# seorim0/DNN-based-Speech-Enhancement-in-the-frequency-domain

Hardware: AMD Instinct MI355X
Metric: train utts/sec (3s@16kHz) DCCRN (higher is better)
Workload: dtype bf16; 1 GPU; DCCRN mask C, SI-SNR, fwd+bwd+Adam, B=32/GPU x 3s@16kHz clips (BASELINE configs[1]); global_batch=32, parallelism=dp1, bn=per-rank statistics, collective=none

## Files before the change

dnn-based-speech-enhancement-in-the-frequency-domain_amd/csrc/bn.hip:

```cpp
#include <hip/hip_runtime.h>
#include <cstdlib>
#include "sefd_desc.h"
#include "tuning.h"
#include "dev_common.h"

namespace sefd {

template <typename T> struct VecIO;
template <> struct VecIO<float> {
  static constexpr int V = 4;
  static __device__ __forceinline__ void load(const char* base, int64_t i, float* o) {
    const float4 v = *reinterpret_cast<const float4*>(base + i * 4);
    o[0] = v.x; o[1] = v.y; o[2] = v.z; o[3] = v.w;
  }
  static __device__ __forceinline__ void store(char* base, int64_t i, const float* o) {
    *reinterpret_cast<float4*>(base + i * 4) = make_float4(o[0], o[1], o[2], o[3]);
  }
};
template <> struct VecIO<bf16_t> {
  static constexpr int V = 8;
  static __device__ __forceinline__ void load(const char* base, int64_t i, float* o) {
    const uint4 v = *reinterpret_cast<const uint4*>(base + i * 2);
    const uint32_t w[4] = {v.x, v.y, v.z, v.w};
#pragma unroll
    for (int k = 0; k < 4; ++k) { o[2 * k] = bf2f(w[k] & 0xffff); o[2 * k + 1] = bf2f(w[k] >> 16); }
  }
  static __device__ __forceinline__ void store(char* base, int64_t i, const float* o) {
    uint4 v;
    v.x = pack_bf16x2(o[0], o[1]); v.y = pack_bf16x2(o[2], o[3]);
    v.z = pack_bf16x2(o[4], o[5]); v.w = pack_bf16x2(o[6], o[7]);
    *reinterpret_cast<uint4*>(base + i * 2) = v;
  }
};

constexpr int kMaxC = kBnMaxC;
static_assert(kMaxC <= 1024, "bn_bwd_reduce_kernel_v: red[512 * V + 8] holds 256 V channels x 2 sums, and C / V chunk columns must fit 256 threads in fp32");

__device__ __forceinline__ void stage_params(float* sp, int C, const float* mi, const float* gamma, const float* beta) {
  for (int c = threadIdx.x; c < C; c += blockDim.x) { sp[c] = mi[c]; sp[C + c] = mi[C + c]; sp[2 * C + c] = gamma[c]; sp[3 * C + c] = beta[c]; }
  __syncthreads();
}

template <typename T>
__global__ __launch_bounds__(256) void bn_apply_kernel_v(const BnApply d, const ArenaBases ab, const int rev) {
  constexpr int V = VecIO<T>::V;
  __shared__ float sp[4 * kMaxC];
  const int C = d.C;
  stage_params(sp, C, reinterpret_cast<const float*>(rp(ab, d.mean_invstd)), reinterpret_cast<const float*>(rp(ab, d.gamma)),
               reinterpret_cast<const float*>(rp(ab, d.beta)));
  const char* y = rp(ab, d.y);
  char* z = rp(ab, d.z);
  const float a = *reinterpret_cast<const float*>(rp(ab, d.slope));
  const int cmask = (C & (C - 1)) == 0 ? C - 1 : -1;
  const int64_t nq = d.R * C / V;
  const int64_t stride = (int64_t)gridDim.x * blockDim.x;
  if (cmask >= 0 && ((stride * V) & cmask) == 0) {
    const int64_t idx0 = blockIdx.x * (int64_t)blockDim.x + threadIdx.x;
    const int c = (int)(((rev ? nq - 1 - idx0 : idx0) * V) & cmask);
    float pm[V], pis[V], pg[V], pb[V];
#pragma unroll
    for (int e = 0; e < V; ++e) { pm[e] = sp[c + e]; pis[e] = sp[C + c + e]; pg[e] = sp[2 * C + c + e]; pb[e] = sp[3 * C + c + e]; }
    for (int64_t qq = idx0; qq < nq; qq += stride) {
      const int64_t q = rev ? nq - 1 - qq : qq;
      float v[V];
      VecIO<T>::load(y, q * V, v);
#pragma unroll
      for (int e = 0; e < V; ++e) {
        const float bn = pg[e] * ((v[e] - pm[e]) * pis[e]) + pb[e];
        v[e] = bn > 0.f ? bn : a * bn;
      }
      VecIO<T>::store(z, q * V, v);
    }
    return;
  }
  for (int64_t q = blockIdx.x * (int64_t)blockDim.x + threadIdx.x; q < nq; q += stride) {
    const int64_t i = q * V;
    const int c = cmask >= 0 ? (int)(i & cmask) : (int)(i % C);
    float v[V];
    VecIO<T>::load(y, i, v);
#pragma unroll
    for (int e = 0; e < V; ++e) {
      const float bn = sp[2 * C + c + e] * ((v[e] - sp[c + e]) * sp[C + c + e]) + sp[3 * C + c + e];
      v[e] = bn > 0.f ? bn : a * bn;
    }
    VecIO<T>::store(z, i, v);
  }
}

template <typename T>
__device__ __forceinline__ void load_dz_v(const BnBwdReduce& d, const char* dz0, const char* dz1, int64_t b, int ql, int c, float* g) {
  constexpr int V = VecIO<T>::V;
#pragma unroll
  for (int e = 0; e < V; ++e) g[e] = 0.f;
  if (ql >= d.skip) VecIO<T>::load(dz0, (b * (d.rpb - d.skip) + ql - d.skip) * d.C + c, g);
  if (dz1) {
    float h[V];
    VecIO<T>::load(dz1, (b * d.rpb + ql) * d.C + c, h);
#pragma unroll
    for (int e = 0; e < V; ++e) g[e] += h[e];
  }
}

template <typename T>
__global__ __launch_bounds__(256) void bn_bwd_reduce_kernel_v(const BnBwdReduce d, const ArenaBases ab, const int rev) {
  constexpr int V = VecIO<T>::V;
  __shared__ float sp[4 * kMaxC];
  __shared__ float red[512 * V + 8];
  const int C = d.C;
  stage_params(sp, C, reinterpret_cast<const float*>(rp(ab, d.mean_invstd)), reinterpret_cast<const float*>(rp(ab, d.gamma)),
               reinterpret_cast<const float*>(rp(ab, d.beta)));
  const char* y = rp(ab, d.y);
  const char* dz0 = rp(ab, d.dz0);
  const char* dz1 = d.dz1.arena >= 0 ? rp(ab, d.dz1) : nullptr;
  const float a = *reinterpret_cast<const float*>(rp(ab, d.slope));
  const int CV = C / V;
  const int nrl = 256 / CV > 0 ? 256 / CV : 1;
  const int rl = threadIdx.x / CV, cc = threadIdx.x - rl * CV;
  float s0[V], s1[V], sa = 0.f;
#pragma unroll
  for (int e = 0; e < V; ++e) { s0[e] = 0.f; s1[e] = 0.f; }
  const int blk = rev ? (int)gridDim.x - 1 - (int)blockIdx.x : (int)blockIdx.x;
  const int64_t row0 = (int64_t)blk * d.rows_per_blk;
  const int64_t row1 = min(d.R, row0 + d.rows_per_blk);
  if (rl < nrl && cc < CV) {
    const int c = cc * V;
    float pm[V], pis[V], pg[V], pb[V];
#pragma unroll
    for (int e = 0; e < V; ++e) { pm[e] = sp[c + e]; pis[e] = sp[C + c + e]; pg[e] = sp[2 * C + c + e]; pb[e] = sp[3 * C + c + e]; }
    int64_t r = row0 + rl;
    int64_t b = r / d.rpb;
    int ql = (int)(r - b * d.rpb);
    auto accumulate = [&](const float* yv, const float* gz) {
#pragma unroll
      for (int e = 0; e < V; ++e) {
        const float xh = (yv[e] - pm[e]) * pis[e];
        const float bn = pg[e] * xh + pb[e];
        const float dbn = bn > 0.f ? gz[e] : a * gz[e];
        sa += bn > 0.f ? 0.f : bn * gz[e];
        s0[e] += dbn;
        s1[e] += dbn * xh;
      }
    };
    auto next_row = [&]() { r += nrl; ql += nrl; while (ql >= d.rpb) { ql -= (int)d.rpb; ++b; } };
    while (r + nrl < row1) {
      float yv0[V], gz0[V], yv1[V], gz1[V];
      VecIO<T>::load(y, r * C + c, yv0);
      load_dz_v<T>(d, dz0, dz1, b, ql, c, gz0);
      next_row();
      VecIO<T>::load(y, r * C + c, yv1);
      load_dz_v<T>(d, dz0, dz1, b, ql, c, gz1);
      next_row();
      accumulate(yv0, gz0);
      accumulate(yv1, gz1);
    }
    if (r < row1) {
      float yv[V], gz[V];
      VecIO<T>::load(y, r * C + c, yv);
      load_dz_v<T>(d, dz0, dz1, b, ql, c, gz);
      accumulate(yv, gz);
    }
#pragma unroll
    for (int e = 0; e < V; ++e) {
      red[(rl * C + c + e) * 2 + 0] = s0[e];
      red[(rl * C + c + e) * 2 + 1] = s1[e];
    }
  }
  __syncthreads();
  float* part = reinterpret_cast<float*>(rp(ab, d.part)) + (int64_t)blk * 3 * C;
  for (int c = threadIdx.x; c < C; c += 256) {
    float t0 = 0.f, t1 = 0.f;
    for (int k = 0; k < nrl; ++k) { t0 += red[(k * C + c) * 2 + 0]; t1 += red[(k * C + c) * 2 + 1]; }
    part[c] = t0;
    part[C + c] = t1;
  }
  __syncthreads();
  sa = wave_sum(sa);
  if ((threadIdx.x & 63) == 0) red[512 * V + (threadIdx.x >> 6)] = sa;
  __syncthreads();
  if (threadIdx.x == 0) part[2 * C] = red[512 * V] + red[512 * V + 1] + red[512 * V + 2] + red[512 * V + 3];
  for (int c = 1 + threadIdx.x; c < C; c += 256) part[2 * C + c] = 0.f;
}

template <typename T>
__global__ __launch_bounds__(256) void bn_bwd_apply_kernel_v(const BnBwdApply d, const ArenaBases ab) {
  constexpr int V = VecIO<T>::V;
  __shared__ float sp[4 * kMaxC];
  __shared__ float st[2 * kMaxC];
  const BnBwdReduce& r = d.r;
  const int C = r.C;
  stage_params(sp, C, reinterpret_cast<const float*>(rp(ab, r.mean_invstd)), reinterpret_cast<const float*>(rp(ab, r.gamma)),
               reinterpret_cast<const float*>(rp(ab, r.beta)));
  const float* tot = reinterpret_cast<const float*>(rp(ab, d.totals));
  const float inv_n = (float)(1.0 / d.count);
  for (int c = threadIdx.x; c < C; c += blockDim.x) { st[c] = tot[c] * inv_n; st[C + c] = tot[C + c] * inv_n; }
  __syncthreads();
  const char* y = rp(ab, r.y);
  const char* dz0 = rp(ab, r.dz0);
  const char* dz1 = r.dz1.arena >= 0 ? rp(ab, r.dz1) : nullptr;
  char* dy = rp(ab, d.dy);
  const float a = *reinterpret_cast<const float*>(rp(ab, r.slope));
  const int64_t b = blockIdx.y;
  const int nq = (int)(r.rpb * C / V);
  const int cmask = (C & (C - 1)) == 0 ? C - 1 : -1;
  const int csh = cmask >= 0 ? __ffs(C) - 1 : 0;
  const int qstride = gridDim.x * blockDim.x;
  if (cmask >= 0 && ((qstride * V) & cmask) == 0) {
    const int c = ((blockIdx.x * blockDim.x + threadIdx.x) * V) & cmask;
    float pm[V], pis[V], pg[V], pb[V], t0[V], t1[V];
#pragma unroll
    for (int e = 0; e < V; ++e) {
      pm[e] = sp[c + e]; pis[e] = sp[C + c + e]; pg[e] = sp[2 * C + c + e]; pb[e] = sp[3 * C + c + e];
      t0[e] = st[c + e]; t1[e] = st[C + c + e];
    }
    for (int q = blockIdx.x * blockDim.x + threadIdx.x; q < nq; q += qstride) {
      const int il = q * V;
      const int ql = il >> csh;
      float yv[V], gz[V], o[V];
      const int64_t gi = b * r.rpb * C + il;
      VecIO<T>::load(y, gi, yv);
      load_dz_v<T>(r, dz0, dz1, b, ql, c, gz);
#pragma unroll
      for (int e = 0; e < V; ++e) {
        const float xh = (yv[e] - pm[e]) * pis[e];
        const float bn = pg[e] * xh + pb[e];
        const float dbn = bn > 0.f ? gz[e] : a * gz[e];
        o[e] = pg[e] * pis[e] * (dbn - t0[e] - xh * t1[e]);
      }
      VecIO<T>::store(dy, gi, o);
    }
    return;
  }
  for (int q = blockIdx.x * blockDim.x + threadIdx.x; q < nq; q += qstride) {
    const int il = q * V;
    const int ql = cmask >= 0 ? (il >> csh) : il / C;
    const int c = il - ql * C;
    float yv[V], gz[V], o[V];
    const int64_t gi = b * r.rpb * C + il;
    VecIO<T>::load(y, gi, yv);
    load_dz_v<T>(r, dz0, dz1, b, ql, c, gz);
#pragma unroll
    for (int e = 0; e < V; ++e) {
      const float xh = (yv[e] - sp[c + e]) * sp[C + c + e];
      const float bn = sp[2 * C + c + e] * xh + sp[3 * C + c + e];
      const float dbn = bn > 0.f ? gz[e] : a * gz[e];
      o[e] = sp[2 * C + c + e] * sp[C + c + e] * (dbn - st[c + e] - xh * st[C + c + e]);
    }
    VecIO<T>::store(dy, gi, o);
  }
}

static inline int gridcap(int64_t n, int cap = 16384) {
  int64_t g = (n + 255) / 256;
  return (int)(g < 1 ? 1 : (g > cap ? cap : g));
}

void launch_bn(const Op& op, const ArenaBases& ab, hipStream_t st) {
  constexpr int rev = 1;
  if (op.kind == OP_BN_APPLY) {
    const BnApply& d = op.bna;
    if (d.dt == DT_BF16) hipLaunchKernelGGL((bn_apply_kernel_v<bf16_t>), dim3(gridcap(d.R * d.C / 8)), dim3(256), 0, st, d, ab, rev);
    else hipLaunchKernelGGL((bn_apply_kernel_v<float>), dim3(gridcap(d.R * d.C / 4)), dim3(256), 0, st, d, ab, rev);
  } else if (op.kind == OP_BN_BWD_REDUCE) {
    const BnBwdReduce& d = op.bnr;
    if (d.dt == DT_BF16) hipLaunchKernelGGL((bn_bwd_reduce_kernel_v<bf16_t>), dim3(d.nblk), dim3(256), 0, st, d, ab, rev);
    else hipLaunchKernelGGL((bn_bwd_reduce_kernel_v<float>), dim3(d.nblk), dim3(256), 0, st, d, ab, rev);
  } else if (op.kind == OP_BN_BWD_APPLY) {
    const BnBwdApply& d = op.bnb;
    const int nb = (int)(d.r.R / d.r.rpb);
    const int v = d.r.dt == DT_BF16 ? 8 : 4;
    int gx = gridcap(d.r.rpb * d.r.C / v, 16384 / (nb > 0 ? nb : 1) + 1);
    if (d.r.dt == DT_BF16) hipLaunchKernelGGL((bn_bwd_apply_kernel_v<bf16_t>), dim3(gx, nb), dim3(256), 0, st, d, ab);
    else hipLaunchKernelGGL((bn_bwd_apply_kernel_v<float>), dim3(gx, nb), dim3(256), 0, st, d, ab);
  }
}

}
```

dnn-based-speech-enhancement-in-the-frequency-domain_amd/csrc/kernels.hip:

```cpp
#include <hip/hip_runtime.h>
#include <algorithm>
#include <mutex>
#include <unordered_map>
#include "sefd_desc.h"
#include "tuning.h"
#include "dev_common.h"

namespace sefd {

static inline int cdiv64(int64_t a, int64_t b) { return (int)((a + b - 1) / b); }
static inline int grid_for(int64_t n, int block = 256, int cap = 8192) {
  int64_t g = (n + block - 1) / block;
  return (int)(g < 1 ? 1 : (g > cap ? cap : g));
}

__global__ void pack_kernel(const Pack d, const ArenaBases ab) {
  const int32_t* tab = reinterpret_cast<const int32_t*>(rp(ab, d.tab));
  const float* src = reinterpret_cast<const float*>(rp(ab, d.src));
  char* dst = rp(ab, d.dst);
  for (int64_t i = blockIdx.x * (int64_t)blockDim.x + threadIdx.x; i < d.n; i += (int64_t)gridDim.x * blockDim.x) {
    float v = 0.f;
    for (int e = 0; e < d.width; ++e) {
      const int32_t t = tab[i * d.width + e];
      if (t > 0) v += src[t - 1];
      else if (t < 0) v -= src[-t - 1];
    }
    st_elem(dst, d.ddt, i, v);
  }
}

__global__ void packmulti_kernel(const PackMulti m, const ArenaBases ab) {
  const Pack d = reinterpret_cast<const Pack*>(rp(ab, m.entries))[blockIdx.y];
  const int32_t* tab = reinterpret_cast<const int32_t*>(rp(ab, d.tab));
  const float* src = reinterpret_cast<const float*>(rp(ab, d.src));
  char* dst = rp(ab, d.dst);
  for (int64_t i = blockIdx.x * (int64_t)blockDim.x + threadIdx.x; i < d.n; i += (int64_t)gridDim.x * blockDim.x) {
    float v = 0.f;
    for (int e = 0; e < d.width; ++e) {
      const int32_t t = tab[i * d.width + e];
      if (t > 0) v += src[t - 1];
      else if (t < 0) v -= src[-t - 1];
    }
    st_elem(dst, d.ddt, i, v);
  }
}

__global__ __launch_bounds__(256) void splitsum_kernel(Unpack d, const ArenaBases ab) {
  __shared__ float4 red[16][16];
  float* part = reinterpret_cast<float*>(rp(ab, d.part));
  if (d.nseg > 0) {
    const int64_t* seg = reinterpret_cast<const int64_t*>(rp(ab, d.start)) + 3 * (int64_t)blockIdx.y;
    part += seg[0];
    d.n = d.sstride = seg[1];
    d.nsplit = (int32_t)seg[2];
  }
  const int ex = threadIdx.x & 15, sy = threadIdx.x >> 4;
  const bool vec = (d.n & 3) == 0 && (d.sstride & 3) == 0 && (reinterpret_cast<uintptr_t>(part) & 15) == 0;
  for (int64_t base = (int64_t)blockIdx.x * 64; base < d.n; base += (int64_t)gridDim.x * 64) {
    const int64_t i = base + ex * 4;
    float4 s = make_float4(0.f, 0.f, 0.f, 0.f);
    if (vec) {
      if (i < d.n)
        for (int k = sy; k < d.nsplit; k += 16) {
          const float4 v = *reinterpret_cast<const float4*>(part + (int64_t)k * d.sstride + i);
          s.x += v.x; s.y += v.y; s.z += v.z; s.w += v.w;
        }
    } else {
      float* sp = &s.x;
      for (int e = 0; e < 4; ++e)
        if (i + e < d.n)
          for (int k = sy; k < d.nsplit; k += 16) sp[e] += part[(int64_t)k * d.sstride + i + e];
    }
    red[sy][ex] = s;
    __syncthreads();
    if (sy == 0) {
      float4 t = red[0][ex];
#pragma unroll
      for (int j = 1; j < 16; ++j) { const float4 v = red[j][ex]; t.x += v.x; t.y += v.y; t.z += v.z; t.w += v.w; }
      if (vec) { if (i < d.n) *reinterpret_cast<float4*>(part + i) = t; }
      else { const float* tp = &t.x; for (int e = 0; e < 4; ++e) if (i + e < d.n) part[i + e] = tp[e]; }
    }
    __syncthreads();
  }
}

__global__ void unpack_kernel(const Unpack d, const ArenaBases ab) {
  const int32_t* start = reinterpret_cast<const int32_t*>(rp(ab, d.start));
  const int32_t* ent = reinterpret_cast<const int32_t*>(rp(ab, d.ent));
  const float* part = reinterpret_cast<const float*>(rp(ab, d.part));
  float* dst = reinterpret_cast<float*>(rp(ab, d.dst));
  for (int64_t j = blockIdx.x * (int64_t)blockDim.x + threadIdx.x; j < d.n; j += (int64_t)gridDim.x * blockDim.x) {
    float v = 0.f;
    for (int e = start[j]; e < start[j + 1]; ++e) {
      const int32_t t = ent[e];
      if (t > 0) v += part[t - 1];
      else if (t < 0) v -= part[-t - 1];
    }
    if (start[j + 1] > start[j]) dst[j] = v;
  }
}

__global__ __launch_bounds__(256) void bn_finalize_kernel(const BnFinalize d, const ArenaBases ab) {
  const int c = blockIdx.x;
  if (d.nblk < 0) {
    if (threadIdx.x == 0) {
      float* mi = reinterpret_cast<float*>(rp(ab, d.mean_invstd));
      mi[c] = reinterpret_cast<const float*>(rp(ab, d.running_mean))[c];
      mi[d.C + c] = 1.f / sqrtf(reinterpret_cast<const float*>(rp(ab, d.running_var))[c] + d.eps);
    }
    return;
  }
  const float* part = reinterpret_cast<const float*>(rp(ab, d.part));
  __shared__ double r1[256], r2[256];
  if (d.mode == 2) {
    if (threadIdx.x == 0) {
      const double* tot = reinterpret_cast<const double*>(rp(ab, d.totals));
      r1[0] = tot[c];
      r2[0] = tot[d.C + c];
    }
  } else {
    double s1 = 0.0, s2 = 0.0;
    const int nsub = d.nsub > 1 ? d.nsub : 1;
    for (int b = threadIdx.x; b < d.nblk; b += 256)
      for (int u = 0; u < nsub; ++u) {
        s1 += part[((int64_t)b * 2 + 0) * d.Cpad + u * d.substride + c];
        s2 += part[((int64_t)b * 2 + 1) * d.Cpad + u * d.substride + c];
      }
    r1[threadIdx.x] = s1;
    r2[threadIdx.x] = s2;
    __syncthreads();
    for (int o = 128; o > 0; o >>= 1) {
      if (threadIdx.x < o) { r1[threadIdx.x] += r1[threadIdx.x + o]; r2[threadIdx.x] += r2[threadIdx.x + o]; }
      __syncthreads();
    }
    if (d.mode == 1) {
      if (threadIdx.x == 0) {
        double* tot = reinterpret_cast<double*>(rp(ab, d.totals));
        tot[c] = r1[0];
        tot[d.C + c] = r2[0];
      }
      return;
    }
  }
  if (threadIdx.x == 0) {
    const double mean = r1[0] / d.count;
    double var = r2[0] / d.count - mean * mean;
    if (var < 0) var = 0;
    float* mi = reinterpret_cast<float*>(rp(ab, d.mean_invstd));
    mi[c] = (float)mean;
    mi[d.C + c] = (float)(1.0 / sqrt(var + (double)d.eps));
    if (d.running_mean.arena >= 0) {
      float* rm = reinterpret_cast<float*>(rp(ab, d.running_mean));
      float* rv = reinterpret_cast<float*>(rp(ab, d.running_var));
      const double unb = var * (d.count / (d.count > 1 ? d.count - 1 : 1));
      rm[c] = (float)((1.0 - d.momentum) * rm[c] + d.momentum * mean);
// ... 389 lines not shown
    float v = 0.f;
    if (k >= 0 && k < d.NF) {
      const float sr = spec[(f * NS + k + 1) * 2], si = spec[(f * NS + k + 1) * 2 + 1];
      v = sqrtf(sr * sr + si * si);
    }
    st_elem(mags, d.dt, i, v);
  }
}

__global__ void specpad_kernel(const Mags d, const ArenaBases ab) {
  const float* spec = reinterpret_cast<const float*>(rp(ab, d.spec));
  char* out = rp(ab, d.mags);
  const int64_t n = d.frames * d.NF * d.MS;
  for (int64_t i = blockIdx.x * (int64_t)blockDim.x + threadIdx.x; i < n; i += (int64_t)gridDim.x * blockDim.x) {
    const int ch = (int)(i % d.MS);
    const int64_t slot = i / d.MS;
    st_elem(out, d.dt, i, ch < 2 ? spec[slot * 2 + ch] : 0.f);
  }
}

__global__ void ola_fwd_kernel(const Ola d, const ArenaBases ab) {
  const float* fr = reinterpret_cast<const float*>(rp(ab, d.frames));
  const float* coff = reinterpret_cast<const float*>(rp(ab, d.coff));
  float* wav = reinterpret_cast<float*>(rp(ab, d.wav));
  const int64_t n = (int64_t)d.B * d.L;
  for (int64_t i = blockIdx.x * (int64_t)blockDim.x + threadIdx.x; i < n; i += (int64_t)gridDim.x * blockDim.x) {
    const int64_t b = i / d.L;
    const int p = (int)(i - b * d.L) + d.trim;
    if (d.Lout > 0 && p - d.trim >= d.Lout) { wav[i] = 0.f; continue; }
    int t1 = p / d.hop; if (t1 > d.T - 1) t1 = d.T - 1;
    int t0 = (p - d.win + d.hop) / d.hop; if (p - d.win + 1 <= 0) t0 = 0;
    float s = 0.f;
    for (int t = t0; t <= t1; ++t) s += fr[((int64_t)b * d.T + t) * d.win + (p - t * d.hop)];
    s = d.noclamp == 1 ? s / coff[p] : s / (coff[p] + 1e-8f);
    wav[i] = d.noclamp ? s : fminf(1.f, fmaxf(-1.f, s));
  }
}
__global__ void ola_bwd_kernel(const Ola d, const ArenaBases ab) {
  const float* coff = reinterpret_cast<const float*>(rp(ab, d.coff));
  const float* wav = reinterpret_cast<const float*>(rp(ab, d.wav));
  const float* dwav = reinterpret_cast<const float*>(rp(ab, d.dwav));
  float* dpad = reinterpret_cast<float*>(rp(ab, d.dpad));
  const int Lp = (d.T - 1) * d.hop + d.win;
  const int64_t n = (int64_t)d.B * Lp;
  for (int64_t i = blockIdx.x * (int64_t)blockDim.x + threadIdx.x; i < n; i += (int64_t)gridDim.x * blockDim.x) {
    const int64_t b = i / Lp;
    const int p = (int)(i - b * Lp);
    float v = 0.f;
    const int s = p - d.trim;
    if (d.noclamp == 2) {
      if (s >= 0 && s < (d.Lout > 0 ? d.Lout : d.L)) v = dwav[b * d.L + s] / (coff[p] + 1e-8f);
    } else if (d.noclamp == 1) {
      if (s >= 0 && s < (d.Lout > 0 ? d.Lout : d.L)) { const float g = dwav[b * d.L + s]; v = fmaf(g, coff[p], g * coff[Lp + p]); }
    } else if (s >= 0 && s < (d.Lout > 0 ? d.Lout : d.L)) {
      const float w = wav[b * d.L + s];
      if (w > -1.f && w < 1.f) v = dwav[b * d.L + s] / (coff[p] + 1e-8f);
    }
    dpad[i] = v;
  }
}

__global__ __launch_bounds__(256) void specout_fwd_kernel(const SpecOut d, const ArenaBases ab) {
  __shared__ float tr[32][33], ti[32][33];
  const float* est = reinterpret_cast<const float*>(rp(ab, d.est));
  float* outr = reinterpret_cast<float*>(rp(ab, d.out_real));
  float* outi = d.mode == 0 ? reinterpret_cast<float*>(rp(ab, d.out_imag)) : nullptr;
  const int NS = d.NF + 1;
  const int b = blockIdx.z, t0 = blockIdx.x * 32, k0 = blockIdx.y * 32;
  const int tx = threadIdx.x & 31, ty = threadIdx.x >> 5;
  for (int r = ty; r < 32; r += 8) {
    const int t = t0 + r, k = k0 + tx;
    float vr = 0.f, vi = 0.f;
    if (t < d.T && k < d.NF) {
      if (d.mode == 2) {
        vr = est[((int64_t)b * d.T + t) * d.NF + k];
      } else {
        const int64_t o = (((int64_t)b * d.T + t) * NS + k + 1) * 2;
        vr = est[o]; vi = est[o + 1];
        if (d.mode == 1) vr = sqrtf(vr * vr + vi * vi);
      }
    }
    tr[r][tx] = vr; ti[r][tx] = vi;
  }
  __syncthreads();
  for (int r = ty; r < 32; r += 8) {
    const int k = k0 + r, t = t0 + tx;
    if (t < d.T && k < d.NF) {
      const int64_t o = ((int64_t)b * d.NF + k) * d.T + t;
      if (d.mode == 3) { outr[2 * o] = tr[tx][r]; outr[2 * o + 1] = ti[tx][r]; }
      else {
        outr[o] = tr[tx][r];
        if (d.mode == 0) outi[o] = ti[tx][r];
      }
    }
  }
}
__global__ __launch_bounds__(256) void specout_bwd_kernel(const SpecOut d, const ArenaBases ab) {
  __shared__ float tr[32][33], ti[32][33];
  float* dest = reinterpret_cast<float*>(rp(ab, d.est));
  const float* gr = reinterpret_cast<const float*>(rp(ab, d.out_real));
  const float* gi = (d.mode == 2 || d.mode == 3) ? nullptr : reinterpret_cast<const float*>(rp(ab, d.out_imag));
  const int NS = d.NF + 1;
  const int b = blockIdx.z, t0 = blockIdx.x * 32, k0 = blockIdx.y * 32;
  const int tx = threadIdx.x & 31, ty = threadIdx.x >> 5;
  for (int r = ty; r < 32; r += 8) {
    const int k = k0 + r, t = t0 + tx;
    float vr = 0.f, vi = 0.f;
    if (t < d.T && k < d.NF) {
      const int64_t o = ((int64_t)b * d.NF + k) * d.T + t;
      if (d.mode == 3) { vr = gr[2 * o]; vi = gr[2 * o + 1]; }
      else { vr = gr[o]; vi = d.mode == 2 ? 0.f : gi[o]; }
    }
    tr[r][tx] = vr; ti[r][tx] = vi;
  }
  __syncthreads();
  for (int r = ty; r < 32; r += 8) {
    const int t = t0 + r, k = k0 + tx;
    if (t < d.T && k < d.NF) {
      if (d.mode == 2) { dest[((int64_t)b * d.T + t) * d.NF + k] = tr[tx][r]; continue; }
      const int64_t o = (((int64_t)b * d.T + t) * NS + k + 1) * 2;
      if (d.accumulate) { dest[o] += tr[tx][r]; dest[o + 1] += ti[tx][r]; }
      else { dest[o] = tr[tx][r]; dest[o + 1] = ti[tx][r]; }
    }
  }
}

__global__ void lstm_refuse_kernel(int* host_word, int* dev_word) { set_status(host_word, dev_word); }

template <int HMAX, bool DIR>
static void launch_lstm_dir(const LstmRec& d, const ArenaBases& ab, hipStream_t st, bool fwd) {
  dim3 grid((d.B + 15) / 16, d.G);
  dim3 block(64 * (d.H / 16));
  if (fwd) {
    const size_t sh = 2 * 16 * (d.H + 2) * sizeof(float);
    hipLaunchKernelGGL((lstm_fwd_kernel<HMAX, DIR>), grid, block, sh, st, d, ab);
  } else {
    const size_t sh = 16 * (4 * d.H + 2) * sizeof(float);
    hipLaunchKernelGGL((lstm_bwd_kernel<HMAX, DIR>), grid, block, sh, st, d, ab);
  }
}

template <int HMAX>
static void launch_lstm(const Op& op, const ArenaBases& ab, hipStream_t st, bool fwd) {
  const LstmRec& d = op.lstm;
  const int mask = lstm_rev_groups(d);
  if (mask != 0 && (d.t0 != 0 || d.t1 != 0 || d.G > 4)) {
    hipLaunchKernelGGL(lstm_refuse_kernel, dim3(1), dim3(1), 0, st, ab.status, ab.dstatus);
    return;
  }
  if (mask != 0) launch_lstm_dir<HMAX, true>(d, ab, st, fwd);
  else launch_lstm_dir<HMAX, false>(d, ab, st, fwd);
}

constexpr int kFinCG = 32, kFinMaxChunks = 64, kFinMaxC = 2048;
struct FinScratch { double* sums; unsigned* tickets; };

static FinScratch fin_scratch(hipStream_t st) {
  static std::mutex mu;
  static std::unordered_map<StreamKey, FinScratch, StreamKeyHash> map;
  std::lock_guard<std::mutex> lk(mu);
  const StreamKey key = stream_key(st);
  auto it = map.find(key);
  if (it != map.end()) return it->second;
  FinScratch f{};
  const size_t nsum = (size_t)(kFinMaxC / kFinCG) * kFinMaxChunks * 3 * kFinCG + kFinMaxC / kFinCG, ntick = kFinMaxC / kFinCG + 1;
  if (hipMalloc(reinterpret_cast<void**>(&f.sums), nsum * sizeof(double)) != hipSuccess ||
      hipMalloc(reinterpret_cast<void**>(&f.tickets), ntick * sizeof(unsigned)) != hipSuccess ||
      hipMemset(f.tickets, 0, ntick * sizeof(unsigned)) != hipSuccess) {
    f.sums = nullptr; f.tickets = nullptr;
    return f;
  }
  map.emplace(key, f);
  return f;
}

template <int NS, bool BWD>
__device__ __forceinline__ bool fin_stage1(const float* part, int nblk, int C, int ld, int rowstride, FinScratch fs, double* out ,
                                           int nsub = 1, int substride = 0) {
  __shared__ double red[8][3][kFinCG];
  __shared__ unsigned ticket;
  const int g = blockIdx.x, k = blockIdx.y, nch = gridDim.y;
  const int cl = threadIdx.x & 31, rl = threadIdx.x >> 5, c = g * kFinCG + cl;
  const int per = (nblk + nch - 1) / nch, b0 = k * per, b1 = min(nblk, b0 + per);
  double s0 = 0.0, s1 = 0.0, s2 = 0.0;
  if (c < C) {
    int b = b0 + rl;
    if (nsub == 1) {
      for (; b + 24 < b1; b += 32) {
        float v0[4], v1[4], v2[4];
#pragma unroll
        for (int u = 0; u < 4; ++u) {
          const float* row = part + (int64_t)(b + 8 * u) * rowstride;
          v0[u] = row[c]; v1[u] = row[ld + c]; v2[u] = BWD ? row[2 * ld + c] : 0.f;
        }
#pragma unroll
        for (int u = 0; u < 4; ++u) { s0 += v0[u]; s1 += v1[u]; if (BWD) s2 += v2[u]; }
      }
    }
    for (; b < b1; b += 8)
      for (int u = 0; u < nsub; ++u) {
        const float* row = part + (int64_t)b * rowstride + u * substride;
        s0 += row[c];
        s1 += row[ld + c];
        if (BWD) s2 += row[2 * ld + c];
      }
  }
  red[rl][0][cl] = s0; red[rl][1][cl] = s1; red[rl][2][cl] = s2;
  __syncthreads();
  double* mine = fs.sums + ((int64_t)g * kFinMaxChunks + k) * 3 * kFinCG;
  if (threadIdx.x < 3 * kFinCG) {
    const int q = threadIdx.x / kFinCG, cc = threadIdx.x % kFinCG;
    double v = 0.0;
    for (int r = 0; r < 8; ++r) v += red[r][q][cc];
    asm volatile("global_store_dwordx2 %0, %1, off sc0 sc1\n\ts_waitcnt vmcnt(0)" ::"v"(mine + q * kFinCG + cc), "v"(v) : "memory");
  }
  __syncthreads();
  if (threadIdx.x == 0) ticket = atomicInc(fs.tickets + g, (unsigned)nch - 1);
  __syncthreads();
  if (ticket != (unsigned)nch - 1) return false;
  if (threadIdx.x < 3 * kFinCG) {
    const int q = threadIdx.x / kFinCG, cc = threadIdx.x % kFinCG;
    const __amdgpu_buffer_rsrc_t r = __builtin_amdgcn_make_buffer_rsrc(fs.sums + (int64_t)g * kFinMaxChunks * 3 * kFinCG, 0,
                                                                       kFinMaxChunks * 3 * kFinCG * 8, 0x00020000);
    double v = 0.0;
    for (int k0 = 0; k0 < nch; k0 += 16) {
      double x[16];
#pragma unroll
      for (int u = 0; u < 16; ++u) {
        const int kk = k0 + u < nch ? k0 + u : nch - 1;
        x[u] = __builtin_bit_cast(double, __builtin_amdgcn_raw_buffer_load_b64(r, (uint32_t)((kk * 3 * kFinCG + q * kFinCG + cc) * 8), 0, 17));
      }
#pragma unroll
      for (int u = 0; u < 16; ++u)
        if (k0 + u < nch) v += x[u];
    }
    out[q * kFinCG + cc] = v;
  }
  __syncthreads();
  return true;
}

__global__ __launch_bounds__(256) void bn_finalize2_kernel(const BnFinalize d, const ArenaBases ab, FinScratch fs) {
  __shared__ double tot[3 * kFinCG];
  if (!fin_stage1<2, false>(reinterpret_cast<const float*>(rp(ab, d.part)), d.nblk, d.C, d.Cpad, 2 * d.Cpad, fs, tot, d.nsub > 1 ? d.nsub : 1, d.substride)) return;
  const int c = blockIdx.x * kFinCG + threadIdx.x;
  if (threadIdx.x < kFinCG && c < d.C) {
    const double mean = tot[threadIdx.x] / d.count;
    double var = tot[kFinCG + threadIdx.x] / d.count - mean * mean;
    if (var < 0) var = 0;
    float* mi = reinterpret_cast<float*>(rp(ab, d.mean_invstd));
    mi[c] = (float)mean;
    mi[d.C + c] = (float)(1.0 / sqrt(var + (double)d.eps));
    if (d.running_mean.arena >= 0) {
      float* rm = reinterpret_cast<float*>(rp(ab, d.running_mean));
      float* rv = reinterpret_cast<float*>(rp(ab, d.running_var));
      const double unb = var * (d.count / (d.count > 1 ? d.count - 1 : 1));
      rm[c] = (float)((1.0 - d.momentum) * rm[c] + d.momentum * mean);
      rv[c] = (float)((1.0 - d.momentum) * rv[c] + d.momentum * unb);
    }
  }
}

__global__ __launch_bounds__(256) void bn_bwd_finalize2_kernel(const BnBwdApply d, const ArenaBases ab, FinScratch fs) {
  __shared__ double tot[3 * kFinCG];
  __shared__ unsigned last;
  const int C = d.r.C, ld = d.r.ldp > 0 ? d.r.ldp : C;
  if (!fin_stage1<3, true>(reinterpret_cast<const float*>(rp(ab, d.r.part)), d.r.nblk, C, ld, 3 * ld, fs, tot)) return;
  const int c = blockIdx.x * kFinCG + threadIdx.x;
  if (threadIdx.x < kFinCG && c < C) {
    float* t = reinterpret_cast<float*>(rp(ab, d.totals));
    t[c] = (float)tot[threadIdx.x];
    t[C + c] = (float)tot[kFinCG + threadIdx.x];
    reinterpret_cast<float*>(rp(ab, d.dbeta))[c] = (float)tot[threadIdx.x];
    reinterpret_cast<float*>(rp(ab, d.dgamma))[c] = (float)tot[kFinCG + threadIdx.x];
  }
  const int ng = gridDim.x;
  double* gsl = fs.sums + (size_t)(kFinMaxC / kFinCG) * kFinMaxChunks * 3 * kFinCG;
  if (threadIdx.x == 0) {
    double v = 0.0;
    for (int cc = 0; cc < kFinCG; ++cc)
      if (blockIdx.x * kFinCG + cc < C) v += tot[2 * kFinCG + cc];
    asm volatile("global_store_dwordx2 %0, %1, off sc0 sc1\n\ts_waitcnt vmcnt(0)" ::"v"(gsl + blockIdx.x), "v"(v) : "memory");
    last = atomicInc(fs.tickets + kFinMaxC / kFinCG, (unsigned)ng - 1) == (unsigned)ng - 1;
    if (last) {
      const __amdgpu_buffer_rsrc_t r = __builtin_amdgcn_make_buffer_rsrc(gsl, 0, (kFinMaxC / kFinCG) * 8, 0x00020000);
      double s = 0.0;
      for (int g = 0; g < ng; ++g) s += __builtin_bit_cast(double, __builtin_amdgcn_raw_buffer_load_b64(r, (uint32_t)(g * 8), 0, 17));
      reinterpret_cast<float*>(rp(ab, d.dslope))[0] = (float)s;
    }
  }
}

static bool fin_two_level(int nblk, int C, hipStream_t st, FinScratch* fs, dim3* grid) {
  if (nblk < 64 || C > kFinMaxC) return false;
  *fs = fin_scratch(st);
  if (!fs->sums) return false;
  const int nch = std::min(kFinMaxChunks, (nblk + 31) / 32);
  *grid = dim3((C + kFinCG - 1) / kFinCG, nch);
  return true;
}

void launch_misc(const Op& op, const ArenaBases& ab, hipStream_t st) {
  switch (op.kind) {
    case OP_PACK:
      hipLaunchKernelGGL(pack_kernel, dim3(grid_for(op.pack.n)), dim3(256), 0, st, op.pack, ab); break;
    case OP_PACKMULTI:
      hipLaunchKernelGGL(packmulti_kernel, dim3(128, op.packm.count), dim3(256), 0, st, op.packm, ab); break;
    case OP_SPLITSUM:
      hipLaunchKernelGGL(splitsum_kernel, dim3((unsigned)std::min<int64_t>((op.unpack.n + 63) / 64, op.unpack.nseg > 0 ? 1024 : 8192), std::max(1, op.unpack.nseg)),
                         dim3(256), 0, st, op.unpack, ab);
      break;
    case OP_UNPACK:
      hipLaunchKernelGGL(unpack_kernel, dim3(grid_for(op.unpack.n)), dim3(256), 0, st, op.unpack, ab); break;
    case OP_BN_FINALIZE: {
      FinScratch fs; dim3 grid;
      if (op.bnf.nblk >= 0 && op.bnf.mode == 0 && fin_two_level(op.bnf.nblk, op.bnf.C, st, &fs, &grid))
        hipLaunchKernelGGL(bn_finalize2_kernel, grid, dim3(256), 0, st, op.bnf, ab, fs);
      else
        hipLaunchKernelGGL(bn_finalize_kernel, dim3(op.bnf.C), dim3(256), 0, st, op.bnf, ab);
      break;
    }
    case OP_BN_APPLY:
    case OP_BN_BWD_REDUCE:
    case OP_BN_BWD_APPLY:
      launch_bn(op, ab, st); break;
    case OP_CBN_STATS: case OP_CBN_FINALIZE: case OP_CBN_APPLY: case OP_CBN_BWD_REDUCE: case OP_CBN_BWD_FINALIZE: case OP_CBN_BWD_APPLY:
      launch_cbn(op, ab, st); break;
    case OP_BN_BWD_FINALIZE: {
      FinScratch fs; dim3 grid;
      if (fin_two_level(op.bnb.r.nblk, op.bnb.r.C, st, &fs, &grid))
        hipLaunchKernelGGL(bn_bwd_finalize2_kernel, grid, dim3(256), 0, st, op.bnb, ab, fs);
      else
        hipLaunchKernelGGL(bn_bwd_finalize_kernel, dim3(op.bnb.r.C), dim3(256), 0, st, op.bnb, ab);
      break;
    }
    case OP_LSTM_FWD:
    case OP_LSTM_BWD: {
      const bool fwd = op.kind == OP_LSTM_FWD;
      if (op.lstm.hdt == DT_BF16 && op.lstm.impl == 1) launch_lstm_rows(op.lstm, ab, st, fwd);
      else if (op.lstm.hdt == DT_BF16 && op.lstm.H > 128) launch_lstm_cluster(op.lstm, ab, st, fwd);
      else if (op.lstm.hdt == DT_BF16) launch_lstm_bf16(op.lstm, ab, st, fwd);
      else if (op.lstm.H <= 64) launch_lstm<64>(op, ab, st, fwd);
      else launch_lstm<128>(op, ab, st, fwd);
      break;
    }
    case OP_COMBINE_FWD:
      hipLaunchKernelGGL(combine_fwd_kernel, dim3(grid_for(op.comb.rows * op.comb.H)), dim3(256), 0, st, op.comb, ab); break;
    case OP_COMBINE_BWD:
      hipLaunchKernelGGL(combine_bwd_kernel, dim3(grid_for(op.comb.rows * op.comb.H)), dim3(256), 0, st, op.comb, ab); break;
    case OP_MASK_FWD:
      hipLaunchKernelGGL(mask_fwd_kernel, dim3(grid_for(op.mask.frames * (op.mask.NF + 1))), dim3(256), 0, st, op.mask, ab); break;
    case OP_MASK_BWD:
      hipLaunchKernelGGL(mask_bwd_kernel, dim3(op.mask.colsum_rows > 0 ? op.mask.colsum_rows : grid_for(op.mask.frames * 2 * op.mask.NF)), dim3(256), 0, st, op.mask, ab); break;
    case OP_OLA_FWD:
      hipLaunchKernelGGL(ola_fwd_kernel, dim3(grid_for((int64_t)op.ola.B * op.ola.L)), dim3(256), 0, st, op.ola, ab); break;
    case OP_OLA_BWD:
      hipLaunchKernelGGL(ola_bwd_kernel, dim3(grid_for((int64_t)op.ola.B * op.ola.L)), dim3(256), 0, st, op.ola, ab); break;
    case OP_SPECOUT_FWD:
    case OP_SPECOUT_BWD: {
      dim3 grid((op.so.T + 31) / 32, (op.so.NF + 31) / 32, op.so.B);
      if (op.kind == OP_SPECOUT_FWD) hipLaunchKernelGGL(specout_fwd_kernel, grid, dim3(256), 0, st, op.so, ab);
      else hipLaunchKernelGGL(specout_bwd_kernel, grid, dim3(256), 0, st, op.so, ab);
      break;
    }
    case OP_SPECPAD:
      hipLaunchKernelGGL(specpad_kernel, dim3(grid_for(op.mags.frames * op.mags.NF * op.mags.MS)), dim3(256), 0, st, op.mags, ab); break;
    case OP_MAGS:
      hipLaunchKernelGGL(mags_kernel, dim3(grid_for(op.mags.frames * op.mags.MS)), dim3(256), 0, st, op.mags, ab); break;
    case OP_SPECCONV: launch_specconv(op.sc, ab, st); break;
    case OP_NCHW_CL: launch_nchw_cl(op.lay, ab, st); break;
    case OP_MEMSET:
      (void)hipMemsetAsync(rp(ab, op.ms.dst), 0, op.ms.bytes, st); break;
    default: launch_fsn(op, ab, st); break;
  }
}

}
```

Measured before the change: 3361 utt/s.

## Batch loads in BN backward reduce and widen two-level finalize reductions

The BN backward reduce kernel is specialised on whether a second gradient input exists. It now reads per-channel params straight from global memory instead of staging them in shared memory, and issues four rows of raw loads before converting and accumulating, which raises memory-level parallelism. The partial fold drops one barrier. The finalize stage uses buffer loads with fixed-size trips, allows more chunks, and spreads the second-level gather across lanes; the slope fold becomes a wave shuffle. This costs more register pressure and more code paths.

Result: no change. 3373 utt/s, median of 6 (+0.3%).

```diff
diff --git a/dnn-based-speech-enhancement-in-the-frequency-domain_amd/csrc/bn.hip b/dnn-based-speech-enhancement-in-the-frequency-domain_amd/csrc/bn.hip
--- a/dnn-based-speech-enhancement-in-the-frequency-domain_amd/csrc/bn.hip
+++ b/dnn-based-speech-enhancement-in-the-frequency-domain_amd/csrc/bn.hip
@@ -9,22 +9,24 @@
 template <typename T> struct VecIO;
 template <> struct VecIO<float> {
   static constexpr int V = 4;
-  static __device__ __forceinline__ void load(const char* base, int64_t i, float* o) {
-    const float4 v = *reinterpret_cast<const float4*>(base + i * 4);
-    o[0] = v.x; o[1] = v.y; o[2] = v.z; o[3] = v.w;
-  }
+  using Raw = float4;
+  static __device__ __forceinline__ Raw ldraw(const char* base, int64_t i) { return *reinterpret_cast<const float4*>(base + i * 4); }
+  static __device__ __forceinline__ void cvt(const Raw& v, float* o) { o[0] = v.x; o[1] = v.y; o[2] = v.z; o[3] = v.w; }
+  static __device__ __forceinline__ void load(const char* base, int64_t i, float* o) { cvt(ldraw(base, i), o); }
   static __device__ __forceinline__ void store(char* base, int64_t i, const float* o) {
     *reinterpret_cast<float4*>(base + i * 4) = make_float4(o[0], o[1], o[2], o[3]);
   }
 };
 template <> struct VecIO<bf16_t> {
   static constexpr int V = 8;
-  static __device__ __forceinline__ void load(const char* base, int64_t i, float* o) {
-    const uint4 v = *reinterpret_cast<const uint4*>(base + i * 2);
+  using Raw = uint4;
+  static __device__ __forceinline__ Raw ldraw(const char* base, int64_t i) { return *reinterpret_cast<const uint4*>(base + i * 2); }
+  static __device__ __forceinline__ void cvt(const Raw& v, float* o) {
     const uint32_t w[4] = {v.x, v.y, v.z, v.w};
 #pragma unroll
     for (int k = 0; k < 4; ++k) { o[2 * k] = bf2f(w[k] & 0xffff); o[2 * k + 1] = bf2f(w[k] >> 16); }
   }
+  static __device__ __forceinline__ void load(const char* base, int64_t i, float* o) { cvt(ldraw(base, i), o); }
   static __device__ __forceinline__ void store(char* base, int64_t i, const float* o) {
     uint4 v;
     v.x = pack_bf16x2(o[0], o[1]); v.y = pack_bf16x2(o[2], o[3]);
@@ -101,18 +103,18 @@
   }
 }
 
-template <typename T>
+constexpr int kRedRows = 4;
+
+template <typename T, bool DZ1>
 __global__ __launch_bounds__(256) void bn_bwd_reduce_kernel_v(const BnBwdReduce d, const ArenaBases ab, const int rev) {
   constexpr int V = VecIO<T>::V;
-  __shared__ float sp[4 * kMaxC];
+  using Raw = typename VecIO<T>::Raw;
+  constexpr int U = kRedRows;
   __shared__ float red[512 * V + 8];
   const int C = d.C;
-  stage_params(sp, C, reinterpret_cast<const float*>(rp(ab, d.mean_invstd)), reinterpret_cast<const float*>(rp(ab, d.gamma)),
-               reinterpret_cast<const float*>(rp(ab, d.beta)));
   const char* y = rp(ab, d.y);
   const char* dz0 = rp(ab, d.dz0);
-  const char* dz1 = d.dz1.arena >= 0 ? rp(ab, d.dz1) : nullptr;
-  const float a = *reinterpret_cast<const float*>(rp(ab, d.slope));
+  const char* dz1 = DZ1 ? rp(ab, d.dz1) : nullptr;
   const int CV = C / V;
   const int nrl = 256 / CV > 0 ? 256 / CV : 1;
   const int rl = threadIdx.x / CV, cc = threadIdx.x - rl * CV;
@@ -124,11 +126,30 @@
   const int64_t row1 = min(d.R, row0 + d.rows_per_blk);
   if (rl < nrl && cc < CV) {
     const int c = cc * V;
+    const int rpb = (int)d.rpb, skip = d.skip;
+    int64_t r = row0 + rl;
+    Raw ry[U], r0[U], r1[U];
+    bool in0[U];
+    if (r + (U - 1) * nrl < row1) {
+#pragma unroll
+      for (int u = 0; u < U; ++u) ry[u] = VecIO<T>::ldraw(y, (r + u * nrl) * C + c);
+    }
     float pm[V], pis[V], pg[V], pb[V];
-#pragma unroll
-    for (int e = 0; e < V; ++e) { pm[e] = sp[c + e]; pis[e] = sp[C + c + e]; pg[e] = sp[2 * C + c + e]; pb[e] = sp[3 * C + c + e]; }
-    int64_t r = row0 + rl;
-    int64_t b = r / d.rpb;
+    {
+      const float* mi = reinterpret_cast<const float*>(rp(ab, d.mean_invstd));
+      const float* gamma = reinterpret_cast<const float*>(rp(ab, d.gamma));
+      const float* beta = reinterpret_cast<const float*>(rp(ab, d.beta));
+#pragma unroll
+      for (int e = 0; e < V; e += 4) {
+        const float4 m4 = *reinterpret_cast<const float4*>(mi + c + e), i4 = *reinterpret_cast<const float4*>(mi + C + c + e);
+        pm[e] = m4.x; pm[e + 1] = m4.y; pm[e + 2] = m4.z; pm[e + 3] = m4.w;
+        pis[e] = i4.x; pis[e + 1] = i4.y; pis[e + 2] = i4.z; pis[e + 3] = i4.w;
+      }
+#pragma unroll
+      for (int e = 0; e < V; ++e) { pg[e] = gamma[c + e]; pb[e] = beta[c + e]; }
+    }
+    const float a = *reinterpret_cast<const float*>(rp(ab, d.slope));
+    int64_t b = (d.R >> 31) == 0 ? (int64_t)((uint32_t)r / (uint32_t)rpb) : r / d.rpb;
     int ql = (int)(r - b * d.rpb);
     auto accumulate = [&](const float* yv, const float* gz) {
 #pragma unroll
@@ -141,42 +162,53 @@
         s1[e] += dbn * xh;
       }
     };
-    auto next_row = [&]() { r += nrl; ql += nrl; while (ql >= d.rpb) { ql -= (int)d.rpb; ++b; } };
-    while (r + nrl < row1) {
-      float yv0[V], gz0[V], yv1[V], gz1[V];
-      VecIO<T>::load(y, r * C + c, yv0);
-      load_dz_v<T>(d, dz0, dz1, b, ql, c, gz0);
-      next_row();
-      VecIO<T>::load(y, r * C + c, yv1);
-      load_dz_v<T>(d, dz0, dz1, b, ql, c, gz1);
-      next_row();
-      accumulate(yv0, gz0);
-      accumulate(yv1, gz1);
-    }
-    if (r < row1) {
-      float yv[V], gz[V];
-      VecIO<T>::load(y, r * C + c, yv);
-      load_dz_v<T>(d, dz0, dz1, b, ql, c, gz);
-      accumulate(yv, gz);
-    }
+    auto trip = [&](const bool full, const bool have_y) {
+      bool ok[U];
+#pragma unroll
+      for (int u = 0; u < U; ++u) {
+        ok[u] = full || r < row1;
+        in0[u] = ok[u] && ql >= skip;
+        if (!have_y && ok[u]) ry[u] = VecIO<T>::ldraw(y, r * C + c);
+        if (in0[u]) r0[u] = VecIO<T>::ldraw(dz0, (b * (rpb - skip) + ql - skip) * C + c);
+        if (DZ1 && ok[u]) r1[u] = VecIO<T>::ldraw(dz1, r * C + c);
+        r += nrl; ql += nrl;
+        while (ql >= rpb) { ql -= rpb; ++b; }
+      }
+#pragma unroll
+      for (int u = 0; u < U; ++u) {
+        if (!ok[u]) continue;
+        float yv[V], gz[V];
+        VecIO<T>::cvt(ry[u], yv);
+#pragma unroll
+        for (int e = 0; e < V; ++e) gz[e] = 0.f;
+        if (in0[u]) VecIO<T>::cvt(r0[u], gz);
+        if (DZ1) {
+          float h[V];
+          VecIO<T>::cvt(r1[u], h);
+#pragma unroll
+          for (int e = 0; e < V; ++e) gz[e] += h[e];
+        }
+        accumulate(yv, gz);
+      }
+    };
+    if (r + (U - 1) * nrl < row1) trip(true, true);
+    while (r + (U - 1) * nrl < row1) trip(true, false);
+    if (r < row1) trip(false, false);
 #pragma unroll
     for (int e = 0; e < V; ++e) {
       red[(rl * C + c + e) * 2 + 0] = s0[e];
       red[(rl * C + c + e) * 2 + 1] = s1[e];
     }
   }
-  __syncthreads();
-  float* part = reinterpret_cast<float*>(rp(ab, d.part)) + (int64_t)blk * 3 * C;
-  for (int c = threadIdx.x; c < C; c += 256) {
-    float t0 = 0.f, t1 = 0.f;
-    for (int k = 0; k < nrl; ++k) { t0 += red[(k * C + c) * 2 + 0]; t1 += red[(k * C + c) * 2 + 1]; }
-    part[c] = t0;
-    part[C + c] = t1;
-  }
-  __syncthreads();
   sa = wave_sum(sa);
   if ((threadIdx.x & 63) == 0) red[512 * V + (threadIdx.x >> 6)] = sa;
   __syncthreads();
+  float* part = reinterpret_cast<float*>(rp(ab, d.part)) + (int64_t)blk * 3 * C;
+  for (int j = threadIdx.x; j < 2 * C; j += 256) {
+    float t = 0.f;
+    for (int k = 0; k < nrl; ++k) t += red[k * 2 * C + j];
+    part[(j & 1) * C + (j >> 1)] = t;
+  }
   if (threadIdx.x == 0) part[2 * C] = red[512 * V] + red[512 * V + 1] + red[512 * V + 2] + red[512 * V + 3];
   for (int c = 1 + threadIdx.x; c < C; c += 256) part[2 * C + c] = 0.f;
 }
@@ -262,8 +294,11 @@
     else hipLaunchKernelGGL((bn_apply_kernel_v<float>), dim3(gridcap(d.R * d.C / 4)), dim3(256), 0, st, d, ab, rev);
   } else if (op.kind == OP_BN_BWD_REDUCE) {
     const BnBwdReduce& d = op.bnr;
-    if (d.dt == DT_BF16) hipLaunchKernelGGL((bn_bwd_reduce_kernel_v<bf16_t>), dim3(d.nblk), dim3(256), 0, st, d, ab, rev);
-    else hipLaunchKernelGGL((bn_bwd_reduce_kernel_v<float>), dim3(d.nblk), dim3(256), 0, st, d, ab, rev);
+    const bool z1 = d.dz1.arena >= 0;
+    if (d.dt == DT_BF16 && z1) hipLaunchKernelGGL((bn_bwd_reduce_kernel_v<bf16_t, true>), dim3(d.nblk), dim3(256), 0, st, d, ab, rev);
+    else if (d.dt == DT_BF16) hipLaunchKernelGGL((bn_bwd_reduce_kernel_v<bf16_t, false>), dim3(d.nblk), dim3(256), 0, st, d, ab, rev);
+    else if (z1) hipLaunchKernelGGL((bn_bwd_reduce_kernel_v<float, true>), dim3(d.nblk), dim3(256), 0, st, d, ab, rev);
+    else hipLaunchKernelGGL((bn_bwd_reduce_kernel_v<float, false>), dim3(d.nblk), dim3(256), 0, st, d, ab, rev);
   } else if (op.kind == OP_BN_BWD_APPLY) {
     const BnBwdApply& d = op.bnb;
     const int nb = (int)(d.r.R / d.r.rpb);
diff --git a/dnn-based-speech-enhancement-in-the-frequency-domain_amd/csrc/kernels.hip b/dnn-based-speech-enhancement-in-the-frequency-domain_amd/csrc/kernels.hip
--- a/dnn-based-speech-enhancement-in-the-frequency-domain_amd/csrc/kernels.hip
+++ b/dnn-based-speech-enhancement-in-the-frequency-domain_amd/csrc/kernels.hip
@@ -1,6 +1,7 @@
 #include <hip/hip_runtime.h>
 #include <algorithm>
 #include <mutex>
+#include <type_traits>
 #include <unordered_map>
 #include "sefd_desc.h"
 #include "tuning.h"
@@ -696,7 +697,8 @@
   else launch_lstm_dir<HMAX, false>(d, ab, st, fwd);
 }
 
-constexpr int kFinCG = 32, kFinMaxChunks = 64, kFinMaxC = 2048;
+constexpr int kFinCG = 32, kFinLanes = 8, kFinTrip = 8 * kFinLanes, kFinMaxChunks = 128, kFinMaxC = kBnMaxC;
+static_assert(kFinMaxChunks <= 16 * kFinLanes, "fin_stage1: a segment lane of the second level holds at most 16 chunks");
 struct FinScratch { double* sums; unsigned* tickets; };
 
 static FinScratch fin_scratch(hipStream_t st) {
@@ -721,63 +723,90 @@
 template <int NS, bool BWD>
 __device__ __forceinline__ bool fin_stage1(const float* part, int nblk, int C, int ld, int rowstride, FinScratch fs, double* out ,
                                            int nsub = 1, int substride = 0) {
-  __shared__ double red[8][3][kFinCG];
+  __shared__ double red[kFinLanes][3][kFinCG];
   __shared__ unsigned ticket;
   const int g = blockIdx.x, k = blockIdx.y, nch = gridDim.y;
   const int cl = threadIdx.x & 31, rl = threadIdx.x >> 5, c = g * kFinCG + cl;
   const int per = (nblk + nch - 1) / nch, b0 = k * per, b1 = min(nblk, b0 + per);
-  double s0 = 0.0, s1 = 0.0, s2 = 0.0;
-  if (c < C) {
-    int b = b0 + rl;
-    if (nsub == 1) {
-      for (; b + 24 < b1; b += 32) {
-        float v0[4], v1[4], v2[4];
-#pragma unroll
-        for (int u = 0; u < 4; ++u) {
-          const float* row = part + (int64_t)(b + 8 * u) * rowstride;
-          v0[u] = row[c]; v1[u] = row[ld + c]; v2[u] = BWD ? row[2 * ld + c] : 0.f;
+  double s[3] = {0.0, 0.0, 0.0};
+  const int64_t span = (int64_t)max(b1 - b0, 0) * rowstride * 4;
+  if (c < C && span > 0) {
+    if (nsub <= 2 && span < ((int64_t)1 << 31)) {
+      const __amdgpu_buffer_rsrc_t rows = __builtin_amdgcn_make_buffer_rsrc(const_cast<float*>(part + (int64_t)b0 * rowstride), 0, (int)span, 0x00020000);
+      auto trips = [&](auto nsub_c) {
+        constexpr int NSUB = decltype(nsub_c)::value, RPT = 8 / NSUB;
+        for (int b = rl; b < b1 - b0; b += kFinLanes * RPT) {
+          float v[NS][8];
+#pragma unroll
+          for (int u = 0; u < RPT; ++u)
+#pragma unroll
+            for (int h = 0; h < NSUB; ++h)
+#pragma unroll
+              for (int q = 0; q < NS; ++q)
+                v[q][u * NSUB + h] = __builtin_bit_cast(float, __builtin_amdgcn_raw_buffer_load_b32(
+                    rows, (uint32_t)(((b + kFinLanes * u) * rowstride + h * substride + q * ld + c) * 4), 0, 0));
+#pragma unroll
+          for (int i = 0; i < 8; ++i)
+#pragma unroll
+            for (int q = 0; q < NS; ++q) s[q] += v[q][i];
         }
-#pragma unroll
-        for (int u = 0; u < 4; ++u) { s0 += v0[u]; s1 += v1[u]; if (BWD) s2 += v2[u]; }
-      }
-    }
-    for (; b < b1; b += 8)
-      for (int u = 0; u < nsub; ++u) {
-        const float* row = part + (int64_t)b * rowstride + u * substride;
-        s0 += row[c];
-        s1 += row[ld + c];
-        if (BWD) s2 += row[2 * ld + c];
-      }
-  }
-  red[rl][0][cl] = s0; red[rl][1][cl] = s1; red[rl][2][cl] = s2;
+      };
+      if (nsub == 1) trips(std::integral_constant<int, 1>());
+      else trips(std::integral_constant<int, 2>());
+    } else {
+      for (int b = b0 + rl; b < b1; b += kFinLanes)
+        for (int u = 0; u < nsub; ++u) {
+          const float* row = part + (int64_t)b * rowstride + u * substride + c;
+#pragma unroll
+          for (int q = 0; q < NS; ++q) s[q] += row[q * ld];
+        }
+    }
+  }
+#pragma unroll
+  for (int q = 0; q < 3; ++q) red[rl][q][cl] = s[q];
   __syncthreads();
   double* mine = fs.sums + ((int64_t)g * kFinMaxChunks + k) * 3 * kFinCG;
-  if (threadIdx.x < 3 * kFinCG) {
+  if (threadIdx.x < NS * kFinCG) {
     const int q = threadIdx.x / kFinCG, cc = threadIdx.x % kFinCG;
     double v = 0.0;
-    for (int r = 0; r < 8; ++r) v += red[r][q][cc];
+    for (int r = 0; r < kFinLanes; ++r) v += red[r][q][cc];
     asm volatile("global_store_dwordx2 %0, %1, off sc0 sc1\n\ts_waitcnt vmcnt(0)" ::"v"(mine + q * kFinCG + cc), "v"(v) : "memory");
   }
   __syncthreads();
   if (threadIdx.x == 0) ticket = atomicInc(fs.tickets + g, (unsigned)nch - 1);
   __syncthreads();
   if (ticket != (unsigned)nch - 1) return false;
-  if (threadIdx.x < 3 * kFinCG) {
-    const int q = threadIdx.x / kFinCG, cc = threadIdx.x % kFinCG;
+  {
+    const int seg = (nch + kFinLanes - 1) / kFinLanes, k0 = rl * seg, k1 = min(nch, k0 + seg);
     const __amdgpu_buffer_rsrc_t r = __builtin_amdgcn_make_buffer_rsrc(fs.sums + (int64_t)g * kFinMaxChunks * 3 * kFinCG, 0,
                                                                        kFinMaxChunks * 3 * kFinCG * 8, 0x00020000);
+    double t[3] = {0.0, 0.0, 0.0};
+    auto gather = [&](auto batch_c) {
+      constexpr int B = decltype(batch_c)::value;
+      double x[NS][B];
+#pragma unroll
+      for (int u = 0; u < B; ++u) {
+        const int kk = k0 + u < k1 ? k0 + u : 0;
+#pragma unroll
+        for (int q = 0; q < NS; ++q)
+          x[q][u] = __builtin_bit_cast(double, __builtin_amdgcn_raw_buffer_load_b64(r, (uint32_t)((kk * 3 * kFinCG + q * kFinCG + cl) * 8), 0, 17));
+      }
+#pragma unroll
+      for (int u = 0; u < B; ++u)
+        if (k0 + u < k1)
+#pragma unroll
+          for (int q = 0; q < NS; ++q) t[q] += x[q][u];
+    };
+    if (seg <= 4) gather(std::integral_constant<int, 4>());
+    else gather(std::integral_constant<int, 16>());
+#pragma unroll
+    for (int q = 0; q < 3; ++q) red[rl][q][cl] = t[q];
+  }
+  __syncthreads();
+  if (threadIdx.x < NS * kFinCG) {
+    const int q = threadIdx.x / kFinCG, cc = threadIdx.x % kFinCG;
     double v = 0.0;
-    for (int k0 = 0; k0 < nch; k0 += 16) {
-      double x[16];
-#pragma unroll
-      for (int u = 0; u < 16; ++u) {
-        const int kk = k0 + u < nch ? k0 + u : nch - 1;
-        x[u] = __builtin_bit_cast(double, __builtin_amdgcn_raw_buffer_load_b64(r, (uint32_t)((kk * 3 * kFinCG + q * kFinCG + cc) * 8), 0, 17));
-      }
-#pragma unroll
-      for (int u = 0; u < 16; ++u)
-        if (k0 + u < nch) v += x[u];
-    }
+    for (int r = 0; r < kFinLanes; ++r) v += red[r][q][cc];
     out[q * kFinCG + cc] = v;
   }
   __syncthreads();
@@ -807,7 +836,6 @@
 
 __global__ __launch_bounds__(256) void bn_bwd_finalize2_kernel(const BnBwdApply d, const ArenaBases ab, FinScratch fs) {
   __shared__ double tot[3 * kFinCG];
-  __shared__ unsigned last;
   const int C = d.r.C, ld = d.r.ldp > 0 ? d.r.ldp : C;
   if (!fin_stage1<3, true>(reinterpret_cast<const float*>(rp(ab, d.r.part)), d.r.nblk, C, ld, 3 * ld, fs, tot)) return;
   const int c = blockIdx.x * kFinCG + threadIdx.x;
@@ -818,29 +846,40 @@
     reinterpret_cast<float*>(rp(ab, d.dbeta))[c] = (float)tot[threadIdx.x];
     reinterpret_cast<float*>(rp(ab, d.dgamma))[c] = (float)tot[kFinCG + threadIdx.x];
   }
-  const int ng = gridDim.x;
+  static_assert(kFinMaxC / kFinCG <= 32, "bn_bwd_finalize2_kernel: one lane per channel group in the slope fold");
+  if ((threadIdx.x >> 6) != 1) return;
+  const int lane = threadIdx.x & 63, ng = gridDim.x;
+  auto fold32 = [](double v) {
+#pragma unroll
+    for (int o = 16; o > 0; o >>= 1) v += __shfl_xor(v, o);
+    return v;
+  };
+  const double share = fold32(lane < kFinCG && blockIdx.x * kFinCG + lane < C ? tot[2 * kFinCG + lane] : 0.0);
+  float* dslope = reinterpret_cast<float*>(rp(ab, d.dslope));
+  if (ng == 1) {
+    if (lane == 0) dslope[0] = (float)share;
+    return;
+  }
   double* gsl = fs.sums + (size_t)(kFinMaxC / kFinCG) * kFinMaxChunks * 3 * kFinCG;
-  if (threadIdx.x == 0) {
-    double v = 0.0;
-    for (int cc = 0; cc < kFinCG; ++cc)
-      if (blockIdx.x * kFinCG + cc < C) v += tot[2 * kFinCG + cc];
-    asm volatile("global_store_dwordx2 %0, %1, off sc0 sc1\n\ts_waitcnt vmcnt(0)" ::"v"(gsl + blockIdx.x), "v"(v) : "memory");
+  unsigned last = 0;
+  if (lane == 0) {
+    asm volatile("global_store_dwordx2 %0, %1, off sc0 sc1\n\ts_waitcnt vmcnt(0)" ::"v"(gsl + blockIdx.x), "v"(share) : "memory");
     last = atomicInc(fs.tickets + kFinMaxC / kFinCG, (unsigned)ng - 1) == (unsigned)ng - 1;
-    if (last) {
-      const __amdgpu_buffer_rsrc_t r = __builtin_amdgcn_make_buffer_rsrc(gsl, 0, (kFinMaxC / kFinCG) * 8, 0x00020000);
-      double s = 0.0;
-      for (int g = 0; g < ng; ++g) s += __builtin_bit_cast(double, __builtin_amdgcn_raw_buffer_load_b64(r, (uint32_t)(g * 8), 0, 17));
-      reinterpret_cast<float*>(rp(ab, d.dslope))[0] = (float)s;
-    }
-  }
-}
-
-static bool fin_two_level(int nblk, int C, hipStream_t st, FinScratch* fs, dim3* grid) {
+  }
+  if (!__shfl(last, 0)) return;
+  const __amdgpu_buffer_rsrc_t r = __builtin_amdgcn_make_buffer_rsrc(gsl, 0, (kFinMaxC / kFinCG) * 8, 0x00020000);
+  const double mine = lane < ng ? __builtin_bit_cast(double, __builtin_amdgcn_raw_buffer_load_b64(r, (uint32_t)(lane * 8), 0, 17)) : 0.0;
+  const double total = fold32(lane < 32 ? mine : 0.0);
+  if (lane == 0) dslope[0] = (float)total;
+}
+
+static int fin_chunks(int64_t units) { return (int)std::min<int64_t>(kFinMaxChunks, (units + kFinTrip - 1) / kFinTrip); }
+
+static bool fin_two_level(int nblk, int nsub, int C, hipStream_t st, FinScratch* fs, dim3* grid) {
   if (nblk < 64 || C > kFinMaxC) return false;
   *fs = fin_scratch(st);
   if (!fs->sums) return false;
-  const int nch = std::min(kFinMaxChunks, (nblk + 31) / 32);
-  *grid = dim3((C + kFinCG - 1) / kFinCG, nch);
+  *grid = dim3((C + kFinCG - 1) / kFinCG, fin_chunks((int64_t)nblk * std::max(nsub, 1)));
   return true;
 }
 
@@ -858,7 +897,7 @@
       hipLaunchKernelGGL(unpack_kernel, dim3(grid_for(op.unpack.n)), dim3(256), 0, st, op.unpack, ab); break;
     case OP_BN_FINALIZE: {
       FinScratch fs; dim3 grid;
-      if (op.bnf.nblk >= 0 && op.bnf.mode == 0 && fin_two_level(op.bnf.nblk, op.bnf.C, st, &fs, &grid))
+      if (op.bnf.nblk >= 0 && op.bnf.mode == 0 && fin_two_level(op.bnf.nblk, op.bnf.nsub, op.bnf.C, st, &fs, &grid))
         hipLaunchKernelGGL(bn_finalize2_kernel, grid, dim3(256), 0, st, op.bnf, ab, fs);
       else
         hipLaunchKernelGGL(bn_finalize_kernel, dim3(op.bnf.C), dim3(256), 0, st, op.bnf, ab);
@@ -872,7 +911,7 @@
       launch_cbn(op, ab, st); break;
     case OP_BN_BWD_FINALIZE: {
       FinScratch fs; dim3 grid;
-      if (fin_two_level(op.bnb.r.nblk, op.bnb.r.C, st, &fs, &grid))
+      if (fin_two_level(op.bnb.r.nblk, 1, op.bnb.r.C, st, &fs, &grid))
         hipLaunchKernelGGL(bn_bwd_finalize2_kernel, grid, dim3(256), 0, st, op.bnb, ab, fs);
       else
         hipLaunchKernelGGL(bn_bwd_finalize_kernel, dim3(op.bnb.r.C), dim3(256), 0, st, op.bnb, ab);
```
